# shivangchopra11/MedMoE

Measured on AMD Instinct MI355X. Metric: image-text pairs/sec at global batch 1024, higher is better.
Workload: dtype bf16; 1 GPU; cfg2: ViT-B/16 + 12-layer text tower (frozen), 8 experts top-2, 224x224x3 + 77 tokens, fwd+bwd+clip+Adam; global_batch=1024, per_gpu_batch=1024, parallelism=dp1

## Files before the change

### medmoe_amd/csrc/embed.hip

```cpp
#include "common.h"

template <typename InT>
__global__ __launch_bounds__(256) void patchify_kernel(const InT* __restrict__ img, bf16_t* __restrict__ out, int B,
                                                       int C, int H, int W, int p, int ld) {
  const int gw = W / p, gh = H / p;
  const long long total = (long long)B * C * H * gw;
  for (long long i = blockIdx.x * 256LL + threadIdx.x; i < total; i += (long long)gridDim.x * 256) {
    const int gx = i % gw;
    long long r = i / gw;
    const int y = r % H; r /= H;
    const int c = r % C;
    const int b = r / C;
    const int gy = y / p, py = y - gy * p;
    const InT* src = img + (((long long)b * C + c) * H + y) * W + gx * p;
    bf16_t* dst = out + ((long long)b * gh * gw + gy * gw + gx) * ld + c * p * p + py * p;
    for (int k = 0; k < p; ++k) {
      if constexpr (sizeof(InT) == 4) dst[k] = f2bf(src[k]); else dst[k] = src[k];
    }
  }
}

extern "C" int medmoe_patchify_ld(const void* img, void* out, int B, int C, int H, int W, int patch, int in_f32, int ld,
                                  hipStream_t stream) {
  if (!img || !out) return MM_ERR_ARG;
  if (B <= 0 || C <= 0 || patch <= 0 || (H % patch) || (W % patch) || ld < C * patch * patch || (ld % 8)) return MM_ERR_SHAPE;
  const long long total = (long long)B * C * H * (W / patch);
  const int grid = (int)min((total + 255) / 256, (long long)256 * 16);
  if (in_f32)
    hipLaunchKernelGGL(patchify_kernel<float>, dim3(grid), dim3(256), 0, stream, (const float*)img, (bf16_t*)out, B, C, H, W, patch, ld);
  else
    hipLaunchKernelGGL(patchify_kernel<bf16_t>, dim3(grid), dim3(256), 0, stream, (const bf16_t*)img, (bf16_t*)out, B, C, H, W, patch, ld);
  return mm_check_launch();
}

extern "C" int medmoe_patchify(const void* img, void* out, int B, int C, int H, int W, int patch, int in_f32,
                               hipStream_t stream) {
  if ((C * patch * patch) % 8) return MM_ERR_SHAPE;
  return medmoe_patchify_ld(img, out, B, C, H, W, patch, in_f32, C * patch * patch, stream);
}

__global__ __launch_bounds__(256) void init_tokens_kernel(bf16_t* __restrict__ x, const float* __restrict__ cls,
                                                          const float* __restrict__ pos, int B, int Nt, int D) {
  const long long total = (long long)B * Nt * D / 4;
  for (long long i = blockIdx.x * 256LL + threadIdx.x; i < total; i += (long long)gridDim.x * 256) {
    const long long e = i * 4;
    const int col = e % D;
    const int t = (e / D) % Nt;
    float4 v = *(const float4*)(pos + (long long)t * D + col);
    if (t == 0) {
      const float4 c = *(const float4*)(cls + col);
      v.x += c.x; v.y += c.y; v.z += c.z; v.w += c.w;
    }
    uint2 o; o.x = pack2bf(v.x, v.y); o.y = pack2bf(v.z, v.w);
    *(uint2*)(x + e) = o;
  }
}

extern "C" int medmoe_init_tokens(void* x, const float* cls, const float* pos, int B, int Nt, int D,
                                  hipStream_t stream) {
  if (!x || !cls || !pos) return MM_ERR_ARG;
  if (B <= 0 || Nt <= 0 || D <= 0 || (D % 4)) return MM_ERR_SHAPE;
  const long long total = (long long)B * Nt * D / 4;
  const int grid = (int)min((total + 255) / 256, (long long)256 * 16);
  hipLaunchKernelGGL(init_tokens_kernel, dim3(grid), dim3(256), 0, stream, (bf16_t*)x, cls, pos, B, Nt, D);
  return mm_check_launch();
}

__global__ __launch_bounds__(256) void pos_cls_grad_kernel(const bf16_t* __restrict__ dx, float* __restrict__ dpos,
                                                           float* __restrict__ dcls, int B, int Nt, int D) {
  const int t = blockIdx.x, col = (blockIdx.y * 256 + threadIdx.x) * 2;
  if (col >= D) return;
  const bf16_t* src = dx + (long long)t * D + col;
  const long long bs = (long long)Nt * D;
  float s0 = 0.f, s1 = 0.f;
  int b = 0;
  for (; b + 8 <= B; b += 8) {
    uint32_t v[8];
#pragma unroll
    for (int u = 0; u < 8; ++u) v[u] = *(const uint32_t*)(src + (b + u) * bs);
#pragma unroll
    for (int u = 0; u < 8; ++u) { s0 += __uint_as_float(v[u] << 16); s1 += __uint_as_float(v[u] & 0xffff0000u); }
  }
  for (; b < B; ++b) {
    const uint32_t v = *(const uint32_t*)(src + b * bs);
    s0 += __uint_as_float(v << 16); s1 += __uint_as_float(v & 0xffff0000u);
  }
  dpos[(long long)t * D + col] += s0; dpos[(long long)t * D + col + 1] += s1;
  if (t == 0) { dcls[col] += s0; dcls[col + 1] += s1; }
}

extern "C" int medmoe_pos_cls_grad(const void* dx, float* dpos, float* dcls, int B, int Nt, int D,
                                   hipStream_t stream) {
  if (!dx || !dpos || !dcls) return MM_ERR_ARG;
  if (B <= 0 || Nt <= 0 || D <= 0 || (D % 2)) return MM_ERR_SHAPE;
  hipLaunchKernelGGL(pos_cls_grad_kernel, dim3(Nt, (D + 511) / 512), dim3(256), 0, stream, (const bf16_t*)dx, dpos,
                     dcls, B, Nt, D);
  return mm_check_launch();
}

__global__ __launch_bounds__(256) void text_embed_ln_kernel(const int* __restrict__ ids, const int* __restrict__ tts,
                                                            const float* __restrict__ word, const float* __restrict__ pos,
                                                            const float* __restrict__ type, const float* __restrict__ gamma,
                                                            const float* __restrict__ beta, bf16_t* __restrict__ out,
                                                            int rows, int T, int D, int vocab, float eps, const int* __restrict__ src_of_row,
                                                            const int* __restrict__ rows_dev) {
  const int lane = threadIdx.x & 63, wid = threadIdx.x >> 6;
  const int n4 = D >> 2;
  if (rows_dev) rows = min(rows, *rows_dev);
  for (int row = blockIdx.x * 4 + wid; row < rows; row += gridDim.x * 4) {
    const int src = src_of_row ? src_of_row[row] : row;
    const int t = src % T;
    int id = ids[src]; id = min(max(id, 0), vocab - 1);
    const int tt = tts ? min(max(tts[src], 0), 1) : 0;
    float4 v[8];
    float s = 0.f;
#pragma unroll
    for (int i = 0; i < 8; ++i) {
      const int c = lane + i * 64;
      if (c < n4) {
        const float4 a = *(const float4*)(word + (long long)id * D + c * 4);
        const float4 p = *(const float4*)(pos + (long long)t * D + c * 4);
        const float4 y = *(const float4*)(type + (long long)tt * D + c * 4);
        v[i] = make_float4(a.x + p.x + y.x, a.y + p.y + y.y, a.z + p.z + y.z, a.w + p.w + y.w);
        s += v[i].x + v[i].y + v[i].z + v[i].w;
      }
    }
    const float mean = wave_sum(s) / (float)D;
    float sq = 0.f;
#pragma unroll
    for (int i = 0; i < 8; ++i)
      if (lane + i * 64 < n4) {
        const float a = v[i].x - mean, b = v[i].y - mean, c = v[i].z - mean, d = v[i].w - mean;
        sq += a * a + b * b + c * c + d * d;
      }
    const float rstd = rsqrtf(wave_sum(sq) / (float)D + eps);
#pragma unroll
    for (int i = 0; i < 8; ++i) {
      const int c = lane + i * 64;
      if (c < n4) {
        const float4 g = *(const float4*)(gamma + c * 4), b = *(const float4*)(beta + c * 4);
        uint2 o;
        o.x = pack2bf((v[i].x - mean) * rstd * g.x + b.x, (v[i].y - mean) * rstd * g.y + b.y);
        o.y = pack2bf((v[i].z - mean) * rstd * g.z + b.z, (v[i].w - mean) * rstd * g.w + b.w);
        *(uint2*)(out + (long long)row * D + c * 4) = o;
      }
    }
  }
}

extern "C" int medmoe_text_embed_ln(const int* ids, const int* type_ids, const float* word, const float* pos,
                                    const float* type, const float* gamma, const float* beta, void* out,
                                    int B, int T, int D, int vocab, float eps, hipStream_t stream) {
  if (!ids || !word || !pos || !type || !gamma || !beta || !out) return MM_ERR_ARG;
  if (B <= 0 || T <= 0 || D <= 0 || (D % 4) || D > 2048 || vocab <= 0) return MM_ERR_SHAPE;
  const int rows = B * T;
  const int grid = min((rows + 3) / 4, 256 * 8);
  hipLaunchKernelGGL(text_embed_ln_kernel, dim3(grid), dim3(256), 0, stream, ids, type_ids, word, pos, type, gamma,
                     beta, (bf16_t*)out, rows, T, D, vocab, eps, (const int*)nullptr, (const int*)nullptr);
  return mm_check_launch();
}

__global__ __launch_bounds__(1024) void text_pack_kernel(const unsigned char* __restrict__ mask, int* __restrict__ tok_row,
                                                         int* __restrict__ src_of_row, int* __restrict__ seq_off, int* __restrict__ count,
                                                         int B, int T) {
  __shared__ int sh[1024];
  const int b = threadIdx.x;
  int n = 0;
  if (b < B)
    for (int t = 0; t < T; ++t) n += mask[b * T + t] ? 1 : 0;
  sh[b] = n;
  __syncthreads();
  for (int o = 1; o < 1024; o <<= 1) {
    const int v = (b >= o) ? sh[b - o] : 0;
    __syncthreads();
    sh[b] += v;
    __syncthreads();
  }
  if (b < B) {
    int r = sh[b] - n;
    seq_off[b] = r;
    for (int t = 0; t < T; ++t) {
      if (mask[b * T + t]) { tok_row[b * T + t] = r; src_of_row[r] = b * T + t; ++r; }
      else tok_row[b * T + t] = -1;
    }
    if (b == B - 1) { seq_off[B] = sh[b]; count[0] = sh[b]; }
  }
}

extern "C" int medmoe_text_pack(const unsigned char* mask, int* tok_row, int* src_of_row, int* seq_off, int* count, int B, int T,
                                hipStream_t stream) {
  if (!mask || !tok_row || !src_of_row || !seq_off || !count) return MM_ERR_ARG;
  if (B <= 0 || B > 1024 || T <= 0) return MM_ERR_SHAPE;
  hipLaunchKernelGGL(text_pack_kernel, dim3(1), dim3(1024), 0, stream, mask, tok_row, src_of_row, seq_off, count, B, T);
  return mm_check_launch();
}

__global__ __launch_bounds__(256) void segment_map_kernel(const void* __restrict__ ids_, int ids64, const unsigned char* __restrict__ is_cont,
                                                          const unsigned char* __restrict__ starts_bracket, int* __restrict__ seg,
                                                          int* __restrict__ cap, int B, int T, int vocab, int sep_id) {
  const int b = blockIdx.x * 256 + threadIdx.x;
  if (b >= B) return;
  auto id_at = [&](int t) -> int {
    const long long v = ids64 ? ((const long long*)ids_)[(long long)b * T + t] : (long long)((const int*)ids_)[(long long)b * T + t];
    return (int)min(max(v, 0ll), (long long)vocab - 1);
  };
  int sep_pos = T;
  for (int t = 0; t < T; ++t)
    if (id_at(t) == sep_id) { sep_pos = t; break; }
  int c = -1, at_sep = 0;
  for (int t = 0; t < T; ++t) {
    const int id = id_at(t);
    const bool st = t == 0 || (t <= sep_pos && !is_cont[id]);
    c += st ? 1 : 0;
    seg[(long long)b * T + t] = c;
    if (t == sep_pos) at_sep = c;
  }
  const int n_words = sep_pos < T ? at_sep + 1 : c;
  int prev = -1, n_real = 0;
  for (int t = 0; t < T; ++t) {
    const int w = seg[(long long)b * T + t];
    const bool keep = t <= sep_pos && w < n_words;
    if (keep && w != prev) {
      n_real += starts_bracket[id_at(t)] ? 0 : 1;
      prev = w;
    }
    if (!keep) seg[(long long)b * T + t] = -1;
  }
  cap[b] = n_real + 1;
}

__global__ __launch_bounds__(256) void segment_map_wave_kernel(const void* __restrict__ ids_, int ids64, const unsigned char* __restrict__ is_cont,
                                                               const unsigned char* __restrict__ starts_bracket, int* __restrict__ seg,
                                                               int* __restrict__ cap, int B, int T, int vocab, int sep_id) {
  const int lane = threadIdx.x & 63;
  const int b = blockIdx.x * 4 + (threadIdx.x >> 6);
  if (b >= B) return;
  int id[2], cont[2], brk[2];
#pragma unroll
  for (int u = 0; u < 2; ++u) {
    const int t = 2 * lane + u;
    id[u] = -1; cont[u] = 0; brk[u] = 0;
    if (t < T) {
      const long long v = ids64 ? ((const long long*)ids_)[(long long)b * T + t] : (long long)((const int*)ids_)[(long long)b * T + t];
      id[u] = (int)min(max(v, 0ll), (long long)vocab - 1);
      cont[u] = is_cont[id[u]]; brk[u] = starts_bracket[id[u]];
    }
  }
  int sep_pos = T;
#pragma unroll
  for (int u = 1; u >= 0; --u) if (2 * lane + u < T && id[u] == sep_id) sep_pos = 2 * lane + u;
#pragma unroll
  for (int m = 32; m > 0; m >>= 1) sep_pos = min(sep_pos, __shfl_xor(sep_pos, m, 64));
  int st[2];
#pragma unroll
  for (int u = 0; u < 2; ++u) { const int t = 2 * lane + u; st[u] = (t < T && (t == 0 || (t <= sep_pos && !cont[u]))) ? 1 : 0; }
  int incl = st[0] + st[1];
#pragma unroll
  for (int m = 1; m < 64; m <<= 1) { const int v = __shfl_up(incl, m, 64); if (lane >= m) incl += v; }
  const int base = incl - st[0] - st[1];
  int c[2] = {base + st[0] - 1, base + st[0] + st[1] - 1};
  const int probe = sep_pos < T ? sep_pos : T - 1;
  int at = (probe >> 1) == lane ? c[probe & 1] : 0;
#pragma unroll
  for (int m = 32; m > 0; m >>= 1) at += __shfl_xor(at, m, 64);
  const int n_words = sep_pos < T ? at + 1 : at;
  int n_real = 0;
#pragma unroll
  for (int u = 0; u < 2; ++u) {
    const int t = 2 * lane + u;
    if (t < T) {
      const bool keep = t <= sep_pos && c[u] < n_words;
      if (keep && st[u] && !brk[u]) n_real += 1;
      seg[(long long)b * T + t] = keep ? c[u] : -1;
    }
  }
#pragma unroll
  for (int m = 32; m > 0; m >>= 1) n_real += __shfl_xor(n_real, m, 64);
  if (lane == 0) cap[b] = n_real + 1;
}

extern "C" int medmoe_segment_map(const void* ids, int ids64, const unsigned char* is_cont, const unsigned char* starts_bracket, int* seg,
                                  int* cap, int B, int T, int vocab, int sep_id, hipStream_t stream) {
  if (!ids || !is_cont || !starts_bracket || !seg || !cap) return MM_ERR_ARG;
  if (B <= 0 || T <= 0 || vocab <= 0 || sep_id < 0 || sep_id >= vocab) return MM_ERR_SHAPE;
  if (T <= 128) {
    hipLaunchKernelGGL(segment_map_wave_kernel, dim3((B + 3) / 4), dim3(256), 0, stream, ids, ids64, is_cont, starts_bracket, seg, cap, B, T,
                       vocab, sep_id);
    return mm_check_launch();
  }
  hipLaunchKernelGGL(segment_map_kernel, dim3((B + 255) / 256), dim3(256), 0, stream, ids, ids64, is_cont, starts_bracket, seg, cap, B, T, vocab,
                     sep_id);
  return mm_check_launch();
}

extern "C" int medmoe_text_embed_ln_packed(const int* ids, const int* type_ids, const float* word, const float* pos, const float* type,
                                           const float* gamma, const float* beta, void* out, int B, int T, int D, int vocab, float eps,
                                           const int* src_of_row, const int* count, hipStream_t stream) {
  if (!ids || !word || !pos || !type || !gamma || !beta || !out || !src_of_row || !count) return MM_ERR_ARG;
  if (B <= 0 || T <= 0 || D <= 0 || (D % 4) || D > 2048 || vocab <= 0) return MM_ERR_SHAPE;
  const int rows = B * T;
  const int grid = min((rows + 3) / 4, 256 * 8);
  hipLaunchKernelGGL(text_embed_ln_kernel, dim3(grid), dim3(256), 0, stream, ids, type_ids, word, pos, type, gamma,
                     beta, (bf16_t*)out, rows, T, D, vocab, eps, src_of_row, count);
  return mm_check_launch();
}

__global__ __launch_bounds__(256) void text_aggregate_kernel(const bf16_t* __restrict__ h0, const bf16_t* __restrict__ h1,
                                                             const bf16_t* __restrict__ h2, const bf16_t* __restrict__ h3,
                                                             int n_layers, const int* __restrict__ seg,
                                                             bf16_t* __restrict__ word16, float* __restrict__ word32,
                                                             float* __restrict__ sent, int T, int D, const int* __restrict__ tok_row) {
  __shared__ int s_seg[256], s_row[256];
  const int b = blockIdx.x, col = blockIdx.y * 512 + threadIdx.x * 2;
  for (int t = threadIdx.x; t < min(T, 256); t += 256) {
    s_seg[t] = seg[b * T + t];
    s_row[t] = tok_row ? tok_row[b * T + t] : b * T + t;
  }
  __syncthreads();
  if (col >= D) return;
  const bf16_t* hs[4] = {h0, h1, h2, h3};
  float a0 = 0.f, a1 = 0.f, s0 = 0.f, s1 = 0.f;
  int cur = -1, written = 0;
  auto flush = [&](int w) {
    const long long o = ((long long)b * T + w) * D + col;
    if (word16) *(uint32_t*)(word16 + o) = pack2bf(a0, a1);
    if (word32) { word32[o] = a0; word32[o + 1] = a1; }
    s0 += a0; s1 += a1;
    a0 = 0.f; a1 = 0.f;
// ... 333 lines not shown
```

### medmoe_amd/csrc/moe.hip

```cpp
#include "common.h"
#include "options.h"

__global__ __launch_bounds__(256) void mean_tokens_kernel(const bf16_t* __restrict__ x, float* __restrict__ out, int Nt,
                                                          int D, int t0, int cnt) {
#pragma clang fp contract(off)
  const int b = blockIdx.x, col = blockIdx.y * 512 + threadIdx.x * 2;
  if (col >= D) return;
  float a0 = 0.f, a1 = 0.f;
  for (int t = t0; t < t0 + cnt; ++t) {
    const uint32_t v = *(const uint32_t*)(x + ((long long)b * Nt + t) * D + col);
    a0 = a0 + __uint_as_float(v << 16);
    a1 = a1 + __uint_as_float(v & 0xffff0000u);
  }
  out[(long long)b * D + col] = a0 / (float)cnt;
  out[(long long)b * D + col + 1] = a1 / (float)cnt;
}

extern "C" int medmoe_mean_tokens(const void* x, float* out, int B, int Nt, int D, int t0, int cnt,
                                  hipStream_t stream) {
  if (!x || !out) return MM_ERR_ARG;
  if (B <= 0 || D <= 0 || (D % 2) || t0 < 0 || cnt <= 0 || t0 + cnt > Nt) return MM_ERR_SHAPE;
  hipLaunchKernelGGL(mean_tokens_kernel, dim3(B, (D + 511) / 512), dim3(256), 0, stream, (const bf16_t*)x, out, Nt, D, t0, cnt);
  return mm_check_launch();
}

__global__ __launch_bounds__(256) void broadcast_tokens_kernel(const float* __restrict__ g, bf16_t* __restrict__ dy,
                                                               int B, int Nt, int D, int t0, int cnt, float scale) {
  const long long total = (long long)B * Nt * D / 4;
  for (long long i = blockIdx.x * 256LL + threadIdx.x; i < total; i += (long long)gridDim.x * 256) {
    const long long e = i * 4;
    const int col = e % D;
    const long long bt = e / D;
    const int t = bt % Nt, b = bt / Nt;
    uint2 o = make_uint2(0u, 0u);
    if (t >= t0 && t < t0 + cnt) {
      const float4 v = *(const float4*)(g + (long long)b * D + col);
      o.x = pack2bf(v.x * scale, v.y * scale); o.y = pack2bf(v.z * scale, v.w * scale);
    }
    *(uint2*)(dy + e) = o;
  }
}

extern "C" int medmoe_broadcast_tokens(const float* g, void* dy, int B, int Nt, int D, int t0, int cnt, float scale,
                                       hipStream_t stream) {
  if (!g || !dy) return MM_ERR_ARG;
  if (B <= 0 || D <= 0 || (D % 4) || t0 < 0 || cnt <= 0 || t0 + cnt > Nt) return MM_ERR_SHAPE;
  const long long total = (long long)B * Nt * D / 4;
  const int grid = (int)min((total + 255) / 256, (long long)256 * 16);
  hipLaunchKernelGGL(broadcast_tokens_kernel, dim3(grid), dim3(256), 0, stream, g, (bf16_t*)dy, B, Nt, D, t0, cnt, scale);
  return mm_check_launch();
}

#define ROUTER_MAX_E 64
__global__ __launch_bounds__(128) void router_fwd_kernel(const float* __restrict__ x, const float* __restrict__ w1,
                                                         const float* __restrict__ b1, const float* __restrict__ w2,
                                                         const float* __restrict__ b2, float* __restrict__ h_out,
                                                         float* __restrict__ probs, int* __restrict__ idx,
                                                         float* __restrict__ gates, int Dv, int Hd, int E, int k) {
#pragma clang fp contract(off)
  extern __shared__ float sm[];
  float* sx = sm; float* sh = sm + Dv; float* sl = sh + Hd;
  const int b = blockIdx.x, j = threadIdx.x;
  for (int c = j; c < Dv; c += blockDim.x) sx[c] = x[(long long)b * Dv + c];
  __syncthreads();
  for (int u = j; u < Hd; u += blockDim.x) {
    float acc = b1[u];
    const float* wr = w1 + (long long)u * Dv;
    for (int c = 0; c < Dv; ++c) { const float pr = sx[c] * wr[c]; acc = acc + pr; }
    acc = fmaxf(acc, 0.f);
    sh[u] = acc;
    h_out[(long long)b * Hd + u] = acc;
  }
  __syncthreads();
  if (j < E) {
    float acc = b2[j];
    const float* wr = w2 + (long long)j * Hd;
    for (int c = 0; c < Hd; ++c) { const float pr = sh[c] * wr[c]; acc = acc + pr; }
    sl[j] = acc;
  }
  __syncthreads();
  if (j < 64) {
    const int e = j;
    const float l = e < E ? sl[e] : -INFINITY;
    const float m = wave_max(l);
    const float ex = e < E ? expf(l - m) : 0.f;
    float s = 0.f;
    for (int q = 0; q < E; ++q) s = s + __shfl(ex, q, 64);
    const float pr = ex / s;
    if (e < E) probs[(long long)b * E + e] = pr;
    float v = e < E ? pr : -2.f;
    float selp[8], selsum = 0.f;
    for (int t = 0; t < k; ++t) {
      float bv = v; int bi = e;
#pragma unroll
      for (int o = 32; o > 0; o >>= 1) {
        const float ov = __shfl_xor(bv, o, 64); const int oi = __shfl_xor(bi, o, 64);
        if (ov > bv || (ov == bv && oi < bi)) { bv = ov; bi = oi; }
      }
      if (e == 0) idx[(long long)b * k + t] = bi;
      selp[t] = bv; selsum += bv;
      if (e == bi) v = -1.f;
    }
    for (int t = 0; t < k; ++t)
      if (e == t) gates[(long long)b * k + t] = (k == 1) ? 1.f : selp[t] / selsum;
  }
}

extern "C" int medmoe_router_fwd(const float* x, const float* w1, const float* b1, const float* w2, const float* b2,
                                 float* h, float* probs, int* idx, float* gates, int B, int Dv, int Hd, int E,
                                 int k, hipStream_t stream) {
  if (!x || !w1 || !b1 || !w2 || !b2 || !h || !probs || !idx || !gates) return MM_ERR_ARG;
  if (B <= 0 || Dv <= 0 || Hd <= 0 || E <= 0 || E > ROUTER_MAX_E || E > 128 || k < 1 || k > 8 || k > E) return MM_ERR_SHAPE;
  const size_t sh = (size_t)(Dv + Hd + E) * sizeof(float);
  hipLaunchKernelGGL(router_fwd_kernel, dim3(B), dim3(128), sh, stream, x, w1, b1, w2, b2, h, probs, idx, gates, Dv, Hd, E, k);
  return mm_check_launch();
}

__global__ __launch_bounds__(128) void router_bwd_kernel(const float* __restrict__ probs, const float* __restrict__ h,
                                                         const float* __restrict__ w2, const int* __restrict__ idx,
                                                         const float* __restrict__ dgates, const int* __restrict__ labels,
                                                         const float* __restrict__ dprobs_ext, float ce_scale,
                                                         float* __restrict__ dlogits,
                                                         float* __restrict__ dh, float* __restrict__ loss_acc,
                                                         int B, int Hd, int E, int k, float* __restrict__ parts = nullptr) {
  __shared__ float sdl[ROUTER_MAX_E];
  const int b = blockIdx.x, j = threadIdx.x;
  if (j == 0) {
    const float* p = probs + (long long)b * E;
    float dp[ROUTER_MAX_E];
    float m = p[0];
    for (int e = 1; e < E; ++e) m = fmaxf(m, p[e]);
    float s = 0.f;
    for (int e = 0; e < E; ++e) { dp[e] = __expf(p[e] - m); s += dp[e]; }
    const int lab = labels ? labels[b] : -1;
    int am = 0;
    for (int e = 1; e < E; ++e) if (p[e] > p[am]) am = e;
    float ce = 0.f;
    for (int e = 0; e < E; ++e) {
      const float q = dp[e] / s;
      if (e == lab) { if (parts) ce = -__logf(q) / (float)B; else atomicAdd(loss_acc, -__logf(q) / (float)B); }
      dp[e] = labels ? ce_scale * (q - (e == lab ? 1.f : 0.f)) : 0.f;
    }
    if (parts) { parts[b] = ce; parts[B + b] = (labels && am == lab) ? 1.f / (float)B : 0.f; }
    else if (labels && am == lab) atomicAdd(loss_acc + 1, 1.f / (float)B);
    if (dprobs_ext)
      for (int e = 0; e < E; ++e) dp[e] += dprobs_ext[(long long)b * E + e];
    if (dgates && k > 1) {
      float ss = 0.f;
      for (int t = 0; t < k; ++t) ss += p[idx[b * k + t]];
      float dot = 0.f;
      for (int t = 0; t < k; ++t) dot += dgates[b * k + t] * p[idx[b * k + t]];
      for (int t = 0; t < k; ++t) dp[idx[b * k + t]] += dgates[b * k + t] / ss - dot / (ss * ss);
    }
    float pd = 0.f;
    for (int e = 0; e < E; ++e) pd += p[e] * dp[e];
    for (int e = 0; e < E; ++e) { sdl[e] = p[e] * (dp[e] - pd); dlogits[(long long)b * E + e] = sdl[e]; }
  }
  __syncthreads();
  for (int u = j; u < Hd; u += blockDim.x) {
    float a = 0.f;
    for (int e = 0; e < E; ++e) a += sdl[e] * w2[(long long)e * Hd + u];
    dh[(long long)b * Hd + u] = h[(long long)b * Hd + u] > 0.f ? a : 0.f;
  }
}

extern "C" int medmoe_router_bwd(const float* probs, const float* h, const float* w2, const int* idx,
                                 const float* dgates, const int* labels, const float* dprobs_ext, float ce_scale,
                                 float* dlogits, float* dh, float* loss_acc, int B, int Hd, int E, int k,
                                 hipStream_t stream) {
  if (!probs || !h || !w2 || !idx || !dlogits || !dh || !loss_acc) return MM_ERR_ARG;
  if (B <= 0 || Hd <= 0 || E <= 0 || E > ROUTER_MAX_E || k < 1 || k > 8) return MM_ERR_SHAPE;
  if (labels && B > 1) ++g_mm_nondet;
  hipLaunchKernelGGL(router_bwd_kernel, dim3(B), dim3(128), 0, stream, probs, h, w2, idx, dgates, labels, dprobs_ext,
                     ce_scale, dlogits, dh, loss_acc, B, Hd, E, k);
  return mm_check_launch();
}

extern "C" int medmoe_router_bwd_det(const float* probs, const float* h, const float* w2, const int* idx,
                                     const float* dgates, const int* labels, const float* dprobs_ext, float ce_scale,
                                     float* dlogits, float* dh, float* loss_acc, int B, int Hd, int E, int k, float* parts,
                                     hipStream_t stream) {
  if (!probs || !h || !w2 || !idx || !dlogits || !dh || !loss_acc || !parts) return MM_ERR_ARG;
  if (B <= 0 || Hd <= 0 || E <= 0 || E > ROUTER_MAX_E || k < 1 || k > 8) return MM_ERR_SHAPE;
  hipLaunchKernelGGL(router_bwd_kernel, dim3(B), dim3(128), 0, stream, probs, h, w2, idx, dgates, labels, dprobs_ext,
                     ce_scale, dlogits, dh, loss_acc, B, Hd, E, k, parts);
  mm_launch_det_sum(parts, B, 2, loss_acc, stream);
  return mm_check_launch();
}

__global__ __launch_bounds__(256) void router_eval_kernel(const float* __restrict__ probs, const int* __restrict__ labels,
                                                          float* __restrict__ loss_acc, int B, int E) {
  __shared__ float sl[256];
  __shared__ int sh[256];
  const int j = threadIdx.x;
  float loss = 0.f;
  int hits = 0;
  for (int b = j; b < B; b += 256) {
    const float* p = probs + (long long)b * E;
    float m = p[0];
    int am = 0;
    for (int e = 1; e < E; ++e) { m = fmaxf(m, p[e]); if (p[e] > p[am]) am = e; }
    float s = 0.f;
    for (int e = 0; e < E; ++e) s += __expf(p[e] - m);
    const int lab = labels[b];
    if (lab >= 0 && lab < E) loss += -__logf(__expf(p[lab] - m) / s) / (float)B;
    hits += am == lab;
  }
  sl[j] = loss; sh[j] = hits;
  __syncthreads();
  for (int o = 128; o > 0; o >>= 1) {
    if (j < o) { sl[j] += sl[j + o]; sh[j] += sh[j + o]; }
    __syncthreads();
  }
  if (j == 0) {
    float acc = 0.f;
    for (int n = 0; n < sh[0]; ++n) acc += 1.f / (float)B;
    loss_acc[0] = sl[0];
    loss_acc[1] = acc;
  }
}

extern "C" int medmoe_router_eval(const float* probs, const int* labels, float* loss_acc, int B, int E, hipStream_t stream) {
  if (!probs || !labels || !loss_acc) return MM_ERR_ARG;
  if (B <= 0 || E <= 0 || E > ROUTER_MAX_E) return MM_ERR_SHAPE;
  hipLaunchKernelGGL(router_eval_kernel, dim3(1), dim3(256), 0, stream, probs, labels, loss_acc, B, E);
  return mm_check_launch();
}

__global__ __launch_bounds__(256) void sgemm_kernel(const float* __restrict__ A, const float* __restrict__ Bm,
                                                    float* __restrict__ C, int M, int N, int K, long long sam,
                                                    long long sak, long long sbk, long long sbn, long long ldc,
                                                    float alpha, float beta) {
  __shared__ float sA[16][65], sB[16][65];
  const int tx = threadIdx.x & 15, ty = threadIdx.x >> 4;
  const int m0 = blockIdx.y * 64, n0 = blockIdx.x * 64;
  float acc[4][4] = {};
  for (int k0 = 0; k0 < K; k0 += 16) {
    for (int i = threadIdx.x; i < 64 * 16; i += 256) {
      const int kk = i & 15, r = i >> 4;
      sA[kk][r] = (m0 + r < M && k0 + kk < K) ? A[(long long)(m0 + r) * sam + (long long)(k0 + kk) * sak] : 0.f;
      sB[kk][r] = (n0 + r < N && k0 + kk < K) ? Bm[(long long)(k0 + kk) * sbk + (long long)(n0 + r) * sbn] : 0.f;
    }
    __syncthreads();
#pragma unroll
    for (int kk = 0; kk < 16; ++kk) {
      float a[4], b[4];
#pragma unroll
      for (int i = 0; i < 4; ++i) { a[i] = sA[kk][ty * 4 + i]; b[i] = sB[kk][tx * 4 + i]; }
#pragma unroll
      for (int i = 0; i < 4; ++i)
#pragma unroll
        for (int jn = 0; jn < 4; ++jn) acc[i][jn] += a[i] * b[jn];
    }
    __syncthreads();
  }
#pragma unroll
  for (int i = 0; i < 4; ++i)
#pragma unroll
    for (int jn = 0; jn < 4; ++jn) {
      const int m = m0 + ty * 4 + i, n = n0 + tx * 4 + jn;
      if (m < M && n < N) {
        float* c = C + (long long)m * ldc + n;
        *c = alpha * acc[i][jn] + (beta != 0.f ? beta * (*c) : 0.f);
      }
    }
}

extern "C" int medmoe_sgemm(const float* A, const float* Bm, float* C, int M, int N, int K, long long sam,
                            long long sak, long long sbk, long long sbn, long long ldc, float alpha, float beta,
                            hipStream_t stream) {
  if (!A || !Bm || !C) return MM_ERR_ARG;
  if (M <= 0 || N <= 0 || K <= 0) return MM_ERR_SHAPE;
  hipLaunchKernelGGL(sgemm_kernel, dim3((N + 63) / 64, (M + 63) / 64), dim3(256), 0, stream, A, Bm, C, M, N, K, sam,
                     sak, sbk, sbn, ldc, alpha, beta);
  return mm_check_launch();
}

__global__ __launch_bounds__(256) void dispatch_kernel(const int* __restrict__ idx, int n_items, int E, int P,
                                                       int* __restrict__ slot_of, int* __restrict__ item_of_slot,
                                                       int* __restrict__ expert_of_slot, int* __restrict__ row_off,
                                                       int* __restrict__ tiles, int* __restrict__ tile_count,
                                                       int max_tiles) {
  __shared__ unsigned short cnt[256][ROUTER_MAX_E];
  __shared__ int off[ROUTER_MAX_E + 1], t128[ROUTER_MAX_E + 1], t256[ROUTER_MAX_E + 1];
  const int tid = threadIdx.x;
  const int per = (n_items + 255) / 256;
  const int lo = min(tid * per, n_items), hi = min(lo + per, n_items);
  for (int e = 0; e < E; ++e) cnt[tid][e] = 0;
  for (int i = lo; i < hi; ++i) cnt[tid][idx[i]] += 1;
  __syncthreads();
  if (tid < E) {
    int run = 0;
    for (int t = 0; t < 256; ++t) { const int c = cnt[t][tid]; cnt[t][tid] = (unsigned short)run; run += c; }
    t128[tid + 1] = run;
  }
  __syncthreads();
  if (tid == 0) {
    off[0] = 0;
    for (int e = 0; e < E; ++e) off[e + 1] = off[e] + t128[e + 1];
    t128[0] = 0; t256[0] = 0;
    for (int e = 0; e < E; ++e) {
      const int rows = (off[e + 1] - off[e]) * P;
      t128[e + 1] = t128[e] + (rows + 127) / 128;
      t256[e + 1] = t256[e] + (rows + 255) / 256;
    }
    tile_count[0] = min(t128[E], max_tiles);
    tile_count[1] = min(t256[E], max_tiles);
  }
  __syncthreads();
  if (tid <= E) row_off[tid] = off[tid] * P;
  for (int i = lo; i < hi; ++i) {
    const int e = idx[i];
    const int s = off[e] + cnt[tid][e]++;
    slot_of[i] = s; item_of_slot[s] = i; expert_of_slot[s] = e;
  }
  int* tiles2 = tiles + max_tiles * 4;
  for (int e = 0; e < E; ++e) {
    const int r0 = off[e] * P, r1 = off[e + 1] * P;
    for (int t = tid; t128[e] + t < min(t128[e + 1], max_tiles); t += 256) {
      int* q = tiles + (t128[e] + t) * 4;
      q[0] = e; q[1] = r0 + t * 128; q[2] = r1; q[3] = 0;
    }
    for (int t = tid; t256[e] + t < min(t256[e + 1], max_tiles); t += 256) {
      int* q = tiles2 + (t256[e] + t) * 4;
      q[0] = e; q[1] = r0 + t * 256; q[2] = r1; q[3] = 0;
    }
  }
}

__global__ __launch_bounds__(256) void rowmap_kernel(const int* __restrict__ item_of_slot, int k, int P, int Nt,
                                                     int R, int* __restrict__ rowmap) {
  for (int r = blockIdx.x * 256 + threadIdx.x; r < R; r += gridDim.x * 256) {
    const int s = r / P, p = r - s * P;
    rowmap[r] = (item_of_slot[s] / k) * Nt + 1 + p;
  }
}

extern "C" int medmoe_dispatch(const int* idx, int B, int k, int E, int P, int Nt, int* slot_of, int* item_of_slot,
                               int* expert_of_slot, int* row_off, int* tiles, int* tile_count, int max_tiles,
                               int* rowmap, hipStream_t stream) {
  if (!idx || !slot_of || !item_of_slot || !expert_of_slot || !row_off || !tiles || !tile_count || !rowmap) return MM_ERR_ARG;
  if (B <= 0 || k < 1 || E < 1 || E > ROUTER_MAX_E || P <= 0 || Nt < P + 1 || (long long)B * k >= 65536) return MM_ERR_SHAPE;
  const int R = B * k * P;
  if (max_tiles < (R + 127) / 128 + E) return MM_ERR_SHAPE;
  hipLaunchKernelGGL(dispatch_kernel, dim3(1), dim3(256), 0, stream, idx, B * k, E, P, slot_of, item_of_slot,
                     expert_of_slot, row_off, tiles, tile_count, max_tiles);
  hipLaunchKernelGGL(rowmap_kernel, dim3(min((R + 255) / 256, 2048)), dim3(256), 0, stream, item_of_slot, k, P, Nt, R, rowmap);
  return mm_check_launch();
}

#define SA_S 4
template <int DCH, int HCH>
__global__ __launch_bounds__(256) void scale_attn_fwd_kernel(const bf16_t* __restrict__ G, const bf16_t* __restrict__ H1,
                                                             const float* __restrict__ w2, const float* __restrict__ b2,
                                                             const int* __restrict__ expert_of_slot, int P,
                                                             bf16_t* __restrict__ out, float* __restrict__ wts, int R,
                                                             int Do, int Dh) {
  const int lane = threadIdx.x & 63, wid = threadIdx.x >> 6;
  for (int r = blockIdx.x * 4 + wid; r < R; r += gridDim.x * 4) {
    const int e = expert_of_slot[r / P];
    float a[SA_S];
#pragma unroll
    for (int s = 0; s < SA_S; ++s) {
      float d = 0.f;
#pragma unroll
      for (int i = 0; i < HCH; ++i) {
        const int c = lane + i * 64;
        if (c * 8 < Dh) {
          const uint4 hv = *(const uint4*)(H1 + ((long long)s * R + r) * Dh + c * 8);
          const float4 w0 = *(const float4*)(w2 + (long long)e * Dh + c * 8), w1 = *(const float4*)(w2 + (long long)e * Dh + c * 8 + 4);
          d += __uint_as_float(hv.x << 16) * w0.x + __uint_as_float(hv.x & 0xffff0000u) * w0.y +
               __uint_as_float(hv.y << 16) * w0.z + __uint_as_float(hv.y & 0xffff0000u) * w0.w +
               __uint_as_float(hv.z << 16) * w1.x + __uint_as_float(hv.z & 0xffff0000u) * w1.y +
               __uint_as_float(hv.w << 16) * w1.z + __uint_as_float(hv.w & 0xffff0000u) * w1.w;
        }
      }
      a[s] = wave_sum(d) + b2[e];
    }
    const float m = fmaxf(fmaxf(a[0], a[1]), fmaxf(a[2], a[3]));
    float den = 0.f;
#pragma unroll
    for (int s = 0; s < SA_S; ++s) { a[s] = __expf(a[s] - m); den += a[s]; }
#pragma unroll
    for (int s = 0; s < SA_S; ++s) a[s] /= den;
    if (lane < SA_S) wts[(long long)r * SA_S + lane] = a[lane];
#pragma unroll
    for (int i = 0; i < DCH; ++i) {
      const int c = lane + i * 64;
      if (c * 8 < Do) {
        float o[8] = {};
#pragma unroll
        for (int s = 0; s < SA_S; ++s) {
          const uint4 gv = *(const uint4*)(G + ((long long)s * R + r) * Do + c * 8);
          const uint32_t w[4] = {gv.x, gv.y, gv.z, gv.w};
#pragma unroll
          for (int q = 0; q < 4; ++q) {
            o[2 * q] += a[s] * __uint_as_float(w[q] << 16);
            o[2 * q + 1] += a[s] * __uint_as_float(w[q] & 0xffff0000u);
          }
        }
        uint4 pk;
        pk.x = pack2bf(o[0], o[1]); pk.y = pack2bf(o[2], o[3]); pk.z = pack2bf(o[4], o[5]); pk.w = pack2bf(o[6], o[7]);
        *(uint4*)(out + (long long)r * Do + c * 8) = pk;
      }
    }
  }
}

extern "C" int medmoe_scale_attn_fwd(const void* G, const void* H1, const float* w2, const float* b2,
                                     const int* expert_of_slot, int P, void* out, float* wts, int R, int Do, int Dh,
                                     hipStream_t stream) {
  if (!G || !H1 || !w2 || !b2 || !expert_of_slot || !out || !wts) return MM_ERR_ARG;
  if (R <= 0 || P <= 0 || (R % P) || (Do % 8) || (Dh % 8) || Do > 1024 || Dh > 512) return MM_ERR_SHAPE;
  const int grid = min((R + 3) / 4, 256 * 8);
  hipLaunchKernelGGL((scale_attn_fwd_kernel<2, 1>), dim3(grid), dim3(256), 0, stream, (const bf16_t*)G, (const bf16_t*)H1,
                     w2, b2, expert_of_slot, P, (bf16_t*)out, wts, R, Do, Dh);
  return mm_check_launch();
}

__global__ __launch_bounds__(256) void combine_fwd_kernel(const bf16_t* __restrict__ eo, const int* __restrict__ slot_of,
                                                          const float* __restrict__ gates, bf16_t* __restrict__ img_l,
                                                          int B, int k, int P, int Do) {
  const int lane = threadIdx.x & 63, wid = threadIdx.x >> 6;
  const int rows = B * P, nch = Do >> 3;
  for (int r = blockIdx.x * 4 + wid; r < rows; r += gridDim.x * 4) {
    const int b = r / P, p = r - b * P;
    for (int c = lane; c < nch; c += 64) {
      float o[8] = {};
      for (int j = 0; j < k; ++j) {
        const float gt = gates[b * k + j];
        const uint4 v = *(const uint4*)(eo + ((long long)slot_of[b * k + j] * P + p) * Do + c * 8);
        const uint32_t w[4] = {v.x, v.y, v.z, v.w};
#pragma unroll
        for (int q = 0; q < 4; ++q) {
          o[2 * q] += gt * __uint_as_float(w[q] << 16);
          o[2 * q + 1] += gt * __uint_as_float(w[q] & 0xffff0000u);
        }
      }
      uint4 pk;
      pk.x = pack2bf(o[0], o[1]); pk.y = pack2bf(o[2], o[3]); pk.z = pack2bf(o[4], o[5]); pk.w = pack2bf(o[6], o[7]);
      *(uint4*)(img_l + (long long)r * Do + c * 8) = pk;
    }
  }
}

extern "C" int medmoe_combine_fwd(const void* expert_out, const int* slot_of, const float* gates, void* img_l, int B,
                                  int k, int P, int Do, hipStream_t stream) {
  if (!expert_out || !slot_of || !gates || !img_l) return MM_ERR_ARG;
  if (B <= 0 || k < 1 || P <= 0 || (Do % 8)) return MM_ERR_SHAPE;
  const int grid = min((B * P + 3) / 4, 256 * 8);
  hipLaunchKernelGGL(combine_fwd_kernel, dim3(grid), dim3(256), 0, stream, (const bf16_t*)expert_out, slot_of, gates,
                     (bf16_t*)img_l, B, k, P, Do);
  return mm_check_launch();
}

constexpr int SA_WAVES = 16;
int g_sa_rows = 0;
template <int DCH, int HCH, bool DET = false>
__global__ __launch_bounds__(SA_WAVES * 64) void scale_attn_bwd_kernel(const bf16_t* __restrict__ d_img_l, const float* __restrict__ d_img_g,
                                                             const bf16_t* __restrict__ G, const bf16_t* __restrict__ H1,
                                                             const float* __restrict__ wts, const float* __restrict__ w2,
                                                             const bf16_t* __restrict__ expert_out,
                                                             const int* __restrict__ expert_of_slot,
                                                             const int* __restrict__ item_of_slot, const float* __restrict__ gates,
                                                             int k, int P, bf16_t* __restrict__ dG, bf16_t* __restrict__ dH1,
                                                             float* __restrict__ dw2, float* __restrict__ db2,
                                                             float* __restrict__ dgate, int R, int Do, int Dh, int rows_per_wave,
                                                             float* __restrict__ rec = nullptr, int wps = 1) {
  const int lane = threadIdx.x & 63, wid = threadIdx.x >> 6;
  const int wave = blockIdx.x * SA_WAVES + wid;
  int r_begin = wave * rows_per_wave, r_end = min(R, r_begin + rows_per_wave);
  float dgs = 0.f;
  if constexpr (DET) {
    const int slot = wave / wps, p0 = (wave - slot * wps) * rows_per_wave;
    if (slot >= R / P) return;
    r_begin = slot * P + p0; r_end = slot * P + min(P, p0 + rows_per_wave);
  }
  float aw2[HCH][8];
#pragma unroll
  for (int i = 0; i < HCH; ++i)
#pragma unroll
    for (int q = 0; q < 8; ++q) aw2[i][q] = 0.f;
  float ab2 = 0.f;
  int cur_e = -1;
  auto flush = [&]() {
    if (cur_e < 0) return;
#pragma unroll
    for (int i = 0; i < HCH; ++i) {
      const int c = lane + i * 64;
      if (c * 8 < Dh)
#pragma unroll
        for (int q = 0; q < 8; ++q) { atomicAdd(dw2 + (long long)cur_e * Dh + c * 8 + q, aw2[i][q]); aw2[i][q] = 0.f; }
    }
    if (lane == 0) atomicAdd(db2 + cur_e, ab2);
    ab2 = 0.f;
  };
  for (int r = r_begin; r < r_end; ++r) {
    const int s_ = r / P, p = r - s_ * P;
    const int e = expert_of_slot[s_];
    if (e != cur_e) { flush(); cur_e = e; }
    const int item = item_of_slot[s_];
    const int b = item / k;
    const float gt = gates[item];
    float dfin[DCH][8];
    float dws[SA_S] = {0.f, 0.f, 0.f, 0.f};
    float dg = 0.f;
#pragma unroll
    for (int i = 0; i < DCH; ++i) {
      const int c = lane + i * 64;
      if (c * 8 < Do) {
        float f[8] = {};
        if (d_img_l) {
          const uint4 v = *(const uint4*)(d_img_l + ((long long)b * P + p) * Do + c * 8);
          const uint32_t w[4] = {v.x, v.y, v.z, v.w};
#pragma unroll
          for (int q = 0; q < 4; ++q) { f[2 * q] = __uint_as_float(w[q] << 16); f[2 * q + 1] = __uint_as_float(w[q] & 0xffff0000u); }
        }
        if (d_img_g) {
          const float4 g0 = *(const float4*)(d_img_g + (long long)b * Do + c * 8), g1 = *(const float4*)(d_img_g + (long long)b * Do + c * 8 + 4);
          const float inv = 1.f / (float)P;
          f[0] += g0.x * inv; f[1] += g0.y * inv; f[2] += g0.z * inv; f[3] += g0.w * inv;
          f[4] += g1.x * inv; f[5] += g1.y * inv; f[6] += g1.z * inv; f[7] += g1.w * inv;
        }
        if (dgate) {
          const uint4 v = *(const uint4*)(expert_out + (long long)r * Do + c * 8);
          const uint32_t w[4] = {v.x, v.y, v.z, v.w};
#pragma unroll
          for (int q = 0; q < 4; ++q) dg += f[2 * q] * __uint_as_float(w[q] << 16) + f[2 * q + 1] * __uint_as_float(w[q] & 0xffff0000u);
        }
#pragma unroll
        for (int q = 0; q < 8; ++q) dfin[i][q] = f[q] * gt;
#pragma unroll
        for (int s = 0; s < SA_S; ++s) {
          const uint4 v = *(const uint4*)(G + ((long long)s * R + r) * Do + c * 8);
          const uint32_t w[4] = {v.x, v.y, v.z, v.w};
#pragma unroll
          for (int q = 0; q < 4; ++q)
            dws[s] += dfin[i][2 * q] * __uint_as_float(w[q] << 16) + dfin[i][2 * q + 1] * __uint_as_float(w[q] & 0xffff0000u);
        }
      }
    }
    float w[SA_S], da[SA_S], wd = 0.f;
#pragma unroll
    for (int s = 0; s < SA_S; ++s) { dws[s] = wave_sum(dws[s]); w[s] = wts[(long long)r * SA_S + s]; wd += w[s] * dws[s]; }
#pragma unroll
    for (int s = 0; s < SA_S; ++s) { da[s] = w[s] * (dws[s] - wd); ab2 += da[s]; }
    if (dgate) {
      dg = wave_sum(dg);
      if constexpr (DET) dgs += dg; else if (lane == 0) atomicAdd(dgate + item, dg);
    }
#pragma unroll
    for (int i = 0; i < DCH; ++i) {
      const int c = lane + i * 64;
      if (c * 8 < Do)
#pragma unroll
        for (int s = 0; s < SA_S; ++s) {
          uint4 pk;
          pk.x = pack2bf(w[s] * dfin[i][0], w[s] * dfin[i][1]); pk.y = pack2bf(w[s] * dfin[i][2], w[s] * dfin[i][3]);
          pk.z = pack2bf(w[s] * dfin[i][4], w[s] * dfin[i][5]); pk.w = pack2bf(w[s] * dfin[i][6], w[s] * dfin[i][7]);
          *(uint4*)(dG + ((long long)s * R + r) * Do + c * 8) = pk;
        }
    }
#pragma unroll
    for (int i = 0; i < HCH; ++i) {
      const int c = lane + i * 64;
      if (c * 8 < Dh) {
        const float4 w0 = *(const float4*)(w2 + (long long)e * Dh + c * 8), w1 = *(const float4*)(w2 + (long long)e * Dh + c * 8 + 4);
        const float wv[8] = {w0.x, w0.y, w0.z, w0.w, w1.x, w1.y, w1.z, w1.w};
#pragma unroll
        for (int s = 0; s < SA_S; ++s) {
          const uint4 hv = *(const uint4*)(H1 + ((long long)s * R + r) * Dh + c * 8);
          const uint32_t hw_[4] = {hv.x, hv.y, hv.z, hv.w};
          float hf[8], o[8];
#pragma unroll
          for (int q = 0; q < 4; ++q) { hf[2 * q] = __uint_as_float(hw_[q] << 16); hf[2 * q + 1] = __uint_as_float(hw_[q] & 0xffff0000u); }
#pragma unroll
          for (int q = 0; q < 8; ++q) { o[q] = hf[q] > 0.f ? da[s] * wv[q] : 0.f; aw2[i][q] += da[s] * hf[q]; }
// ... 266 lines not shown
```

Before: 4779 pairs/s.

## Vectorize patchify and rewrite fp32 SGEMM with split-K, double-buffered tiles and thin path

Adds a vectorized patchify kernel that moves 8 elements per thread with 16-byte loads and stores when the patch size and pointer alignment allow it. Replaces the fp32 SGEMM with a split-K kernel in which each of 4 wavefronts handles a K slice. Each wavefront double-buffers its LDS tiles, uses vectorized float4 loads chosen by stride layout, computes an 8x8 register tile with packed FMAs, and the partial sums are reduced through LDS. Adds a thin-M kernel for M<=8 that splits K across 16 wavefronts. These target small fp32 GEMMs (router/CLIP) and the patchify copy, which are minor parts of a step dominated by bf16 GEMMs.

New measurement: 4796 pairs/s (median of 6 runs). Within noise of the previous version (+0.4%).

```diff
diff --git a/medmoe_amd/csrc/embed.hip b/medmoe_amd/csrc/embed.hip
--- a/medmoe_amd/csrc/embed.hip
+++ b/medmoe_amd/csrc/embed.hip
@@ -20,10 +20,48 @@
   }
 }
 
+template <typename InT>
+__global__ __launch_bounds__(256) void patchify_vec_kernel(const InT* __restrict__ img, bf16_t* __restrict__ out, int B,
+                                                           int C, int H, int W, int p, int ld) {
+  const int gw = W / p, gh = H / p, p8 = p >> 3;
+  const int per_c = p * p8, per_patch = C * per_c;
+  const long long total = (long long)B * gh * gw * per_patch;
+  for (long long i = blockIdx.x * 256LL + threadIdx.x; i < total; i += (long long)gridDim.x * 256) {
+    const long long patch = i / per_patch;
+    const int q = (int)(i - patch * per_patch);
+    const int c = q / per_c, r = q - c * per_c;
+    const int py = r / p8, px = (r - py * p8) * 8;
+    const int gx = (int)(patch % gw);
+    const long long t = patch / gw;
+    const int gy = (int)(t % gh), b = (int)(t / gh);
+    const InT* src = img + (((long long)b * C + c) * H + gy * p + py) * W + gx * p + px;
+    bf16_t* dst = out + patch * ld + c * p * p + py * p + px;
+    if constexpr (sizeof(InT) == 4) {
+      const float4 v0 = *(const float4*)src, v1 = *(const float4*)(src + 4);
+      const bf16_t h[8] = {f2bf(v0.x), f2bf(v0.y), f2bf(v0.z), f2bf(v0.w), f2bf(v1.x), f2bf(v1.y), f2bf(v1.z), f2bf(v1.w)};
+      uint4 o;
+      o.x = (uint32_t)h[0] | ((uint32_t)h[1] << 16); o.y = (uint32_t)h[2] | ((uint32_t)h[3] << 16);
+      o.z = (uint32_t)h[4] | ((uint32_t)h[5] << 16); o.w = (uint32_t)h[6] | ((uint32_t)h[7] << 16);
+      *(uint4*)dst = o;
+    } else {
+      *(uint4*)dst = *(const uint4*)src;
+    }
+  }
+}
+
 extern "C" int medmoe_patchify_ld(const void* img, void* out, int B, int C, int H, int W, int patch, int in_f32, int ld,
                                   hipStream_t stream) {
   if (!img || !out) return MM_ERR_ARG;
   if (B <= 0 || C <= 0 || patch <= 0 || (H % patch) || (W % patch) || ld < C * patch * patch || (ld % 8)) return MM_ERR_SHAPE;
+  if ((patch % 8) == 0 && (((uintptr_t)img | (uintptr_t)out) & 15) == 0) {
+    const long long pieces = (long long)B * C * H * W / 8;
+    const int vgrid = (int)min((pieces + 255) / 256, (long long)256 * 16);
+    if (in_f32)
+      hipLaunchKernelGGL(patchify_vec_kernel<float>, dim3(vgrid), dim3(256), 0, stream, (const float*)img, (bf16_t*)out, B, C, H, W, patch, ld);
+    else
+      hipLaunchKernelGGL(patchify_vec_kernel<bf16_t>, dim3(vgrid), dim3(256), 0, stream, (const bf16_t*)img, (bf16_t*)out, B, C, H, W, patch, ld);
+    return mm_check_launch();
+  }
   const long long total = (long long)B * C * H * (W / patch);
   const int grid = (int)min((total + 255) / 256, (long long)256 * 16);
   if (in_f32)
diff --git a/medmoe_amd/csrc/moe.hip b/medmoe_amd/csrc/moe.hip
--- a/medmoe_amd/csrc/moe.hip
+++ b/medmoe_amd/csrc/moe.hip
@@ -227,43 +227,194 @@
   return mm_check_launch();
 }
 
-__global__ __launch_bounds__(256) void sgemm_kernel(const float* __restrict__ A, const float* __restrict__ Bm,
-                                                    float* __restrict__ C, int M, int N, int K, long long sam,
-                                                    long long sak, long long sbk, long long sbn, long long ldc,
-                                                    float alpha, float beta) {
-  __shared__ float sA[16][65], sB[16][65];
-  const int tx = threadIdx.x & 15, ty = threadIdx.x >> 4;
-  const int m0 = blockIdx.y * 64, n0 = blockIdx.x * 64;
-  float acc[4][4] = {};
-  for (int k0 = 0; k0 < K; k0 += 16) {
-    for (int i = threadIdx.x; i < 64 * 16; i += 256) {
-      const int kk = i & 15, r = i >> 4;
-      sA[kk][r] = (m0 + r < M && k0 + kk < K) ? A[(long long)(m0 + r) * sam + (long long)(k0 + kk) * sak] : 0.f;
-      sB[kk][r] = (n0 + r < N && k0 + kk < K) ? Bm[(long long)(k0 + kk) * sbk + (long long)(n0 + r) * sbn] : 0.f;
+#define SG_T 64
+#define SG_K 16
+#define SG_W 4
+struct SgOperand { const float* p; long long s_edge, s_k; int n_edge, mode; };
+
+__device__ __forceinline__ void sg_load(const SgOperand& o, int e0, int k0, int k_end, int lane, float4 (&r)[4]) {
+  if (o.mode == 1) {
+    const int kq = (lane & 3) * 4 + k0;
+#pragma unroll
+    for (int i = 0; i < 4; ++i) {
+      const int e = e0 + (lane >> 2) + 16 * i;
+      const float* src = o.p + (long long)e * o.s_edge + kq;
+      r[i] = make_float4(0.f, 0.f, 0.f, 0.f);
+      if (e < o.n_edge) {
+        if (kq + 3 < k_end) r[i] = *(const float4*)src;
+        else {
+          if (kq < k_end) r[i].x = src[0];
+          if (kq + 1 < k_end) r[i].y = src[1];
+          if (kq + 2 < k_end) r[i].z = src[2];
+        }
+      }
+    }
+  } else if (o.mode == 2) {
+    const int e = e0 + (lane & 15) * 4;
+#pragma unroll
+    for (int i = 0; i < 4; ++i) {
+      const int k = k0 + (lane >> 4) + 4 * i;
+      const float* src = o.p + (long long)k * o.s_k + e;
+      r[i] = make_float4(0.f, 0.f, 0.f, 0.f);
+      if (k < k_end) {
+        if (e + 3 < o.n_edge) r[i] = *(const float4*)src;
+        else {
+          if (e < o.n_edge) r[i].x = src[0];
+          if (e + 1 < o.n_edge) r[i].y = src[1];
+          if (e + 2 < o.n_edge) r[i].z = src[2];
+        }
+      }
+    }
+  } else {
+    const int e = e0 + lane;
+#pragma unroll
+    for (int i = 0; i < 4; ++i) {
+      float v[4];
+#pragma unroll
+      for (int j = 0; j < 4; ++j) {
+        const int k = k0 + 4 * i + j;
+        v[j] = (e < o.n_edge && k < k_end) ? o.p[(long long)e * o.s_edge + (long long)k * o.s_k] : 0.f;
+      }
+      r[i] = make_float4(v[0], v[1], v[2], v[3]);
+    }
+  }
+}
+
+__device__ __forceinline__ void sg_store(float* s, int mode, int lane, const float4 (&r)[4]) {
+  if (mode == 1) {
+    const int kq = lane & 3;
+#pragma unroll
+    for (int i = 0; i < 4; ++i) {
+      const int col = ((lane >> 2) + 16 * i + 16 * kq) & 63;
+      s[(kq * 4 + 0) * SG_T + col] = r[i].x; s[(kq * 4 + 1) * SG_T + col] = r[i].y;
+      s[(kq * 4 + 2) * SG_T + col] = r[i].z; s[(kq * 4 + 3) * SG_T + col] = r[i].w;
+    }
+  } else if (mode == 2) {
+#pragma unroll
+    for (int i = 0; i < 4; ++i) {
+      const int k = (lane >> 4) + 4 * i;
+      *(float4*)(s + k * SG_T + (((lane & 15) * 4 + 16 * (k >> 2)) & 63)) = r[i];
+    }
+  } else {
+#pragma unroll
+    for (int i = 0; i < 4; ++i) {
+      const int col = (lane + 16 * i) & 63;
+      s[(4 * i + 0) * SG_T + col] = r[i].x; s[(4 * i + 1) * SG_T + col] = r[i].y;
+      s[(4 * i + 2) * SG_T + col] = r[i].z; s[(4 * i + 3) * SG_T + col] = r[i].w;
+    }
+  }
+}
+
+__global__ __launch_bounds__(SG_W * 64) void sgemm_kernel(SgOperand oa, SgOperand ob, float* __restrict__ C, int K, int k_slice, long long ldc,
+                                                          float alpha, float beta) {
+  __shared__ __attribute__((aligned(16))) float smem[SG_W * 2 * 2 * SG_K * SG_T];
+  const int lane = threadIdx.x & 63, wid = threadIdx.x >> 6;
+  const int ty = lane >> 3, tx = lane & 7;
+  const int m0 = blockIdx.y * SG_T, n0 = blockIdx.x * SG_T;
+  const int k_begin = wid * k_slice, k_end = min(K, k_begin + k_slice);
+  const int steps = k_slice / SG_K;
+  float* sw = smem + wid * (2 * 2 * SG_K * SG_T);
+  f32x2_t acc[8][4];
+#pragma unroll
+  for (int i = 0; i < 8; ++i)
+#pragma unroll
+    for (int j = 0; j < 4; ++j) acc[i][j] = (f32x2_t){0.f, 0.f};
+  float4 ra[4], rb[4];
+  sg_load(oa, m0, k_begin, k_end, lane, ra);
+  sg_load(ob, n0, k_begin, k_end, lane, rb);
+  sg_store(sw, oa.mode, lane, ra);
+  sg_store(sw + SG_K * SG_T, ob.mode, lane, rb);
+  __syncthreads();
+  for (int s = 0; s < steps; ++s) {
+    const float* cA = sw + (s & 1) * (2 * SG_K * SG_T);
+    const float* cB = cA + SG_K * SG_T;
+    if (s + 1 < steps) {
+      sg_load(oa, m0, k_begin + (s + 1) * SG_K, k_end, lane, ra);
+      sg_load(ob, n0, k_begin + (s + 1) * SG_K, k_end, lane, rb);
+    }
+#pragma unroll 1
+    for (int kq = 0; kq < SG_K / 4; ++kq) {
+      const int rot = 16 * kq;
+      const float* pa0 = cA + kq * 4 * SG_T + ((ty * 4 + rot) & 63), *pa1 = cA + kq * 4 * SG_T + ((ty * 4 + 32 + rot) & 63);
+      const float* pb0 = cB + kq * 4 * SG_T + ((tx * 4 + rot) & 63), *pb1 = cB + kq * 4 * SG_T + ((tx * 4 + 32 + rot) & 63);
+#pragma unroll
+      for (int kk = 0; kk < 4; ++kk) {
+        const float4 a0 = *(const float4*)(pa0 + kk * SG_T), a1 = *(const float4*)(pa1 + kk * SG_T);
+        const float4 b0 = *(const float4*)(pb0 + kk * SG_T), b1 = *(const float4*)(pb1 + kk * SG_T);
+        const float a[8] = {a0.x, a0.y, a0.z, a0.w, a1.x, a1.y, a1.z, a1.w};
+        const f32x2_t b[4] = {{b0.x, b0.y}, {b0.z, b0.w}, {b1.x, b1.y}, {b1.z, b1.w}};
+#pragma unroll
+        for (int i = 0; i < 8; ++i)
+#pragma unroll
+          for (int j = 0; j < 4; ++j) acc[i][j] = __builtin_elementwise_fma((f32x2_t){a[i], a[i]}, b[j], acc[i][j]);
+      }
+    }
+    if (s + 1 < steps) {
+      float* nA = sw + ((s + 1) & 1) * (2 * SG_K * SG_T);
+      sg_store(nA, oa.mode, lane, ra);
+      sg_store(nA + SG_K * SG_T, ob.mode, lane, rb);
     }
     __syncthreads();
-#pragma unroll
-    for (int kk = 0; kk < 16; ++kk) {
-      float a[4], b[4];
-#pragma unroll
-      for (int i = 0; i < 4; ++i) { a[i] = sA[kk][ty * 4 + i]; b[i] = sB[kk][tx * 4 + i]; }
-#pragma unroll
-      for (int i = 0; i < 4; ++i)
-#pragma unroll
-        for (int jn = 0; jn < 4; ++jn) acc[i][jn] += a[i] * b[jn];
-    }
-    __syncthreads();
-  }
-#pragma unroll
-  for (int i = 0; i < 4; ++i)
-#pragma unroll
-    for (int jn = 0; jn < 4; ++jn) {
-      const int m = m0 + ty * 4 + i, n = n0 + tx * 4 + jn;
-      if (m < M && n < N) {
+  }
+  if (wid > 0) {
+#pragma unroll
+    for (int i = 0; i < 8; ++i)
+#pragma unroll
+      for (int j = 0; j < 8; ++j) smem[((wid - 1) * 64 + i * 8 + j) * 64 + lane] = acc[i][j >> 1][j & 1];
+  }
+  __syncthreads();
+  if (wid > 0) return;
+#pragma unroll
+  for (int i = 0; i < 8; ++i) {
+    const int m = m0 + (i >> 2) * 32 + ty * 4 + (i & 3);
+#pragma unroll
+    for (int j = 0; j < 8; ++j) {
+      const int n = n0 + (j >> 2) * 32 + tx * 4 + (j & 3);
+      float v = acc[i][j >> 1][j & 1];
+#pragma unroll
+      for (int w = 0; w < SG_W - 1; ++w) v += smem[(w * 64 + i * 8 + j) * 64 + lane];
+      if (m < oa.n_edge && n < ob.n_edge) {
         float* c = C + (long long)m * ldc + n;
-        *c = alpha * acc[i][jn] + (beta != 0.f ? beta * (*c) : 0.f);
-      }
-    }
+        *c = alpha * v + (beta != 0.f ? beta * (*c) : 0.f);
+      }
+    }
+  }
+}
+
+#define SGT_W 16
+#define SGT_M 8
+__global__ __launch_bounds__(SGT_W * 64) void sgemm_thin_kernel(SgOperand oa, SgOperand ob, float* __restrict__ C, int K, int k_slice,
+                                                                long long ldc, float alpha, float beta) {
+  __shared__ float red[SGT_W - 1][SGT_M][64];
+  const int lane = threadIdx.x & 63, wid = threadIdx.x >> 6;
+  const int n = blockIdx.x * 64 + lane, M = oa.n_edge;
+  const bool on = n < ob.n_edge;
+  const int k_begin = wid * k_slice, k_end = min(K, k_begin + k_slice);
+  const float* bp = ob.p + (long long)(on ? n : 0) * ob.s_edge;
+  float acc[SGT_M];
+#pragma unroll
+  for (int m = 0; m < SGT_M; ++m) acc[m] = 0.f;
+#pragma unroll 4
+  for (int k = k_begin; k < k_end; ++k) {
+    const float b = on ? bp[(long long)k * ob.s_k] : 0.f;
+#pragma unroll
+    for (int m = 0; m < SGT_M; ++m)
+      if (m < M) acc[m] += oa.p[(long long)m * oa.s_edge + (long long)k * oa.s_k] * b;
+  }
+  if (wid > 0) {
+#pragma unroll
+    for (int m = 0; m < SGT_M; ++m) red[wid - 1][m][lane] = acc[m];
+  }
+  __syncthreads();
+  if (wid > 0 || !on) return;
+#pragma unroll
+  for (int m = 0; m < SGT_M; ++m) {
+    if (m >= M) break;
+    float v = acc[m];
+    for (int w = 0; w < SGT_W - 1; ++w) v += red[w][m][lane];
+    float* c = C + (long long)m * ldc + n;
+    *c = alpha * v + (beta != 0.f ? beta * (*c) : 0.f);
+  }
 }
 
 extern "C" int medmoe_sgemm(const float* A, const float* Bm, float* C, int M, int N, int K, long long sam,
@@ -271,8 +422,21 @@
                             hipStream_t stream) {
   if (!A || !Bm || !C) return MM_ERR_ARG;
   if (M <= 0 || N <= 0 || K <= 0) return MM_ERR_SHAPE;
-  hipLaunchKernelGGL(sgemm_kernel, dim3((N + 63) / 64, (M + 63) / 64), dim3(256), 0, stream, A, Bm, C, M, N, K, sam,
-                     sak, sbk, sbn, ldc, alpha, beta);
+  auto mode = [](const float* p, long long s_edge, long long s_k) {
+    if (((uintptr_t)p & 15) != 0) return 0;
+    if (s_k == 1 && s_edge % 4 == 0) return 1;
+    if (s_edge == 1 && s_k % 4 == 0) return 2;
+    return 0;
+  };
+  const SgOperand oa = {A, sam, sak, M, mode(A, sam, sak)}, ob = {Bm, sbn, sbk, N, mode(Bm, sbn, sbk)};
+  if (M <= SGT_M) {
+    const int ks = (K + SGT_W - 1) / SGT_W;
+    hipLaunchKernelGGL(sgemm_thin_kernel, dim3((N + 63) / 64), dim3(SGT_W * 64), 0, stream, oa, ob, C, K, ks, ldc, alpha, beta);
+    return mm_check_launch();
+  }
+  const int k_slice = ((K + SG_W - 1) / SG_W + SG_K - 1) / SG_K * SG_K;
+  hipLaunchKernelGGL(sgemm_kernel, dim3((N + SG_T - 1) / SG_T, (M + SG_T - 1) / SG_T), dim3(SG_W * 64), 0, stream, oa, ob, C, K, k_slice, ldc,
+                     alpha, beta);
   return mm_check_launch();
 }
 
```
